# TritonDataCenter/dragnet

Measured on AMD Instinct MI355X. Metric: NDJSON records/sec (whole node), krill filter + 2-field breakdown (req.method,res.statusCode), higher is better.
Workload: dtype uint8; 1 GPU; model=dn scan: filter eq(req.method,GET) + breakdown req.method,res.statusCode, global_batch=4743501, seq_len=226, parallelism=dp1

## Files before the change

dragnet_amd/ops/hip/ext.hip:

```cpp

#include <torch/extension.h>
#include <cstdlib>
#include <cstring>
#include <c10/hip/HIPStream.h>

#include "scan_kernels.hip"

namespace dn {

namespace {

#define CHECK_GPU(t) TORCH_CHECK((t).is_cuda(), #t " must be on GPU")

constexpr size_t LDS_MAX = 160 * 1024;

hipStream_t current_stream() {
  return c10::hip::getCurrentHIPStream().stream();
}

template <class... KArgs, class... Args>
void launch(const char* what, void (*kernel)(KArgs...), dim3 grid,
            dim3 block, size_t lds, Args&&... args) {
  hipLaunchKernelGGL(kernel, grid, block, lds, current_stream(),
                     std::forward<Args>(args)...);
  hipError_t err = hipGetLastError();
  TORCH_CHECK(err == hipSuccess, what, " launch failed: ",
              hipGetErrorString(err));
}

uint32_t grid_for(uint64_t n) {
  return (uint32_t)std::min<uint64_t>((n + BLOCK - 1) / BLOCK, 2048);
}

int env_int(const char* name, int dflt) {
  const char* v = getenv(name);
  return v ? atoi(v) : dflt;
}

torch::Tensor tensor_at(const py::dict& d, const char* key) {
  return py::cast<torch::Tensor>(d[key]);
}

size_t lds_bytes(int64_t nf, int64_t nm, int64_t ns, bool columnar) {
  return LdsLayout((int)nf, (int)nm, columnar ? 0 : (int)ns, !columnar)
      .total;
}

using ScanKernel = void (*)(ScanArgs);

ScanKernel linear_kernel(int mw) {
  switch (mw) {
    case 2: return scan_kernel_mw<2>;
    case 3: return scan_kernel_mw<3>;
    case 4: return scan_kernel_mw<4>;
    case 5: return scan_kernel_mw<5>;
    case 6: return scan_kernel_mw<6>;
    default: return scan_kernel;
  }
}

ScanKernel xpose_kernel(int mw, int xg) {
  if (xg == 32) return scan_kernel_x<4, 5>;
  if (xg == 128) return scan_kernel_x<4, 7>;
  switch (mw) {
    case 2: return scan_kernel_x<2, 6>;
    case 3: return scan_kernel_x<3, 6>;
    case 5: return scan_kernel_x<5, 6>;
    default: return scan_kernel_x<4, 6>;
  }
}

}

void newline_index(torch::Tensor data, int64_t start, int64_t n,
                   torch::Tensor seg_scratch,
                   torch::Tensor pos_out, torch::Tensor total_out) {
  CHECK_GPU(data);
  int64_t span = n - (start & ~(int64_t)15);
  uint32_t nseg = (uint32_t)((span + NL_SEG - 1) / NL_SEG);
  TORCH_CHECK((int64_t)nseg <= seg_scratch.numel(),
              "seg_scratch too small");
  if (span <= 0) {
    total_out.zero_();
    return;
  }
  const uint8_t* d = (const uint8_t*)data.data_ptr();
  uint32_t* segs = (uint32_t*)seg_scratch.data_ptr();
  uint32_t blocks = (nseg + 3) / 4;
  launch("newline_count", newline_count_kernel, dim3(blocks), dim3(256), 0,
         d, (uint32_t)start, (uint32_t)n, segs, nseg);
  launch("newline_scan", newline_scan_kernel, dim3(1), dim3(1024), 0,
         segs, nseg, (uint32_t*)total_out.data_ptr());
  launch("newline_write", newline_write_kernel, dim3(blocks), dim3(256), 0,
         d, (uint32_t)start, (uint32_t)n, segs, nseg,
         (uint32_t*)pos_out.data_ptr(), (uint32_t)pos_out.numel());
}

torch::Tensor col_descs_host(std::vector<int64_t> kinds,
                             std::vector<torch::Tensor> nums,
                             std::vector<torch::Tensor> soffs,
                             std::vector<torch::Tensor> slens) {
  int nf = (int)kinds.size();
  auto out = torch::zeros({(long)(nf * sizeof(ColDesc))},
                          torch::dtype(torch::kUInt8));
  ColDesc* d = (ColDesc*)out.data_ptr();
  for (int f = 0; f < nf; f++) {
    d[f].kind = (int32_t)kinds[f];
    d[f].num = kinds[f] == 1 ? (const double*)nums[f].data_ptr()
                             : nullptr;
    d[f].soff = kinds[f] == 2 ? (const uint32_t*)soffs[f].data_ptr()
                              : nullptr;
    d[f].slen = kinds[f] == 2 ? (const uint32_t*)slens[f].data_ptr()
                              : nullptr;
  }
  return out;
}

void xpose_build(torch::Tensor data, torch::Tensor sstart,
                 torch::Tensor slen, torch::Tensor wbase,
                 int64_t n_slots, int64_t gran_log, torch::Tensor xb) {
  CHECK_GPU(data);
  CHECK_GPU(xb);
  uint32_t nw = (uint32_t)(n_slots >> 6);
  TORCH_CHECK(wbase.numel() >= (long)nw + 1, "wbase needs nw+1 rows");
  uint32_t blocks = (nw + 3) / 4;
  launch("xpose_build", xpose_build_kernel, dim3(blocks), dim3(256), 0,
         (const uint8_t*)data.data_ptr(),
         (const uint32_t*)sstart.data_ptr(),
         (const uint32_t*)slen.data_ptr(),
         (const unsigned long long*)wbase.data_ptr(),
         (uint32_t)n_slots, (int)gran_log, (uint8_t*)xb.data_ptr());
}

class ScanState {
 public:
  ScanState(py::dict plan, std::vector<torch::Tensor> states,
            std::vector<torch::Tensor> keys,
            std::vector<torch::Tensor> counts,
            std::vector<torch::Tensor> partials, py::dict sdict,
// ... 10 lines not shown
    StrDict& sd = args_.sdict;
    NumDict& nd = args_.ndict;
    P.field_sigs = (const uint64_t*)ptr(plan, "field_sigs");
    P.nf = (int)owned_.back().numel();
    P.comp_slot = (const int32_t*)ptr(plan, "comp_slot");
    P.nf_match = py::cast<int>(plan["nf_match"]);
    P.sig_bloom = (uint64_t)py::cast<int64_t>(plan["sig_bloom"]);
    P.prog_nodes = (const int32_t*)ptr(plan, "prog_nodes");
    P.prog_bounds = (const int32_t*)ptr(plan, "prog_bounds");
    P.const_meta = (const int32_t*)ptr(plan, "const_meta");
    P.const_dvals = (const double*)ptr(plan, "const_dvals");
    P.const_bytes = (const uint8_t*)ptr(plan, "const_bytes");
    P.synth_slots = (const int32_t*)ptr(plan, "synth_slots");
    P.ns = py::cast<int>(plan["n_synth"]);
    P.metric_rows = (const int32_t*)ptr(plan, "metric_rows");
    P.nm = (int)(owned_.back().numel() / 8);
    P.synth_req = (const int32_t*)ptr(plan, "synth_req");
    P.bd_rows = (const int32_t*)ptr(plan, "bd_rows");
    P.bd_steps = (const double*)ptr(plan, "bd_steps");
    P.value_slot = py::cast<int>(plan["value_slot"]);
    P.fields_slot = py::cast<int>(plan["fields_slot"]);
    P.fields_parent_sig =
        (uint64_t)py::cast<int64_t>(plan["fields_parent_sig"]);
    args_.data_format_skinner = py::cast<bool>(plan["skinner"]) ? 1 : 0;

    sd_state_ = tensor_at(sdict, "state");
    sd_data_ = tensor_at(sdict, "data");
    sd_used_ = tensor_at(sdict, "used");
    sd_next_ = tensor_at(sdict, "next");
    sd.state = (uint32_t*)sd_state_.data_ptr();
    sd.hash = (uint64_t*)ptr(sdict, "hash");
    sd.id = (uint32_t*)ptr(sdict, "id");
    sd.off = (uint32_t*)ptr(sdict, "off");
    sd.len = (uint32_t*)ptr(sdict, "len");
    sd.nslots = (uint32_t)sd_state_.numel();
    sd.data = (uint8_t*)sd_data_.data_ptr();
    sd.data_cap = (uint32_t)sd_data_.numel();
    sd.data_used = (uint32_t*)sd_used_.data_ptr();
    sd.next_id = (uint32_t*)sd_next_.data_ptr();

    nd_state_ = tensor_at(ndict, "state");
    nd_next_ = tensor_at(ndict, "next");
    nd.state = (uint32_t*)nd_state_.data_ptr();
    nd.bits = (uint64_t*)ptr(ndict, "bits");
    nd.id = (uint32_t*)ptr(ndict, "id");
    nd.nslots = (uint32_t)nd_state_.numel();
    nd.next_id = (uint32_t*)nd_next_.data_ptr();

    size_t nm = states_.size();
    TORCH_CHECK((int)nm == P.nm && keys_.size() == nm &&
                    counts_.size() == nm &&
                    (partials_.empty() || partials_.size() == nm),
                "one table (and partial) per metric");
    tables_.resize(nm);
    for (size_t m = 0; m < nm; m++) {
      AggTable& t = tables_[m];
      t.state = (uint32_t*)states_[m].data_ptr();
      t.keys = (uint32_t*)keys_[m].data_ptr();
      t.count = (double*)counts_[m].data_ptr();
      t.nslots = (uint32_t)states_[m].numel();
      t.partial = nullptr;
      t.prows = 0;
      t.pad_ = 0;
      if (!partials_.empty()) {
        TORCH_CHECK(partials_[m].size(1) == (long)t.nslots,
                    "partial width != nslots");
        t.partial = (double*)partials_[m].data_ptr();
        t.prows = (uint32_t)partials_[m].size(0);
      }
    }
    for (auto* group : {&states_, &keys_, &counts_, &partials_, &owned_})
      for (auto& t : *group) CHECK_GPU(t);
    for (auto* t : {&sd_state_, &sd_data_, &sd_used_, &sd_next_,
                    &nd_state_, &nd_next_})
      CHECK_GPU(*t);
    auto host = torch::empty({(long)(nm * sizeof(AggTable))},
                             torch::dtype(torch::kUInt8));
    memcpy(host.data_ptr(), tables_.data(), nm * sizeof(AggTable));
    table_descs_ = host.to(counters_.device());
    args_.tables = (AggTable*)table_descs_.data_ptr();
    args_.counters = (unsigned long long*)counters_.data_ptr();

    int mw = env_int("DRAGNET_MIN_WAVES", 4);
    linear_ = linear_kernel(mw);
    xpose_ = xpose_kernel(mw, env_int("DRAGNET_XGRAN", 64));

    lds_ = lds_bytes(P.nf, P.nm, P.ns, false);
    TORCH_CHECK(lds_ <= LDS_MAX, "plan needs too much LDS: ", lds_);
    int tile_req = env_int("DRAGNET_LDS_STAGE", 0);
    if (tile_req != 0) {
      size_t avail = (LDS_MAX - lds_ - 256) & ~(size_t)15;
      tile_cap_ = (tile_req < 0) ? avail
                                 : std::min((size_t)tile_req, avail);
      if (tile_cap_ > 100 * 1024) tile_cap_ = 100 * 1024;
      if (tile_cap_ < 24 * 1024) tile_cap_ = 0;
    }
    args_.tile_cap = (uint32_t)tile_cap_;
  }

  void scan(torch::Tensor data, torch::Tensor nl_pos,
            torch::Tensor nlines, int64_t first_start) {
    CHECK_GPU(data);
    CHECK_GPU(nl_pos);
    ScanArgs A = args_;
    A.data = (const uint8_t*)data.data_ptr();
    A.nl_pos = (const uint32_t*)nl_pos.data_ptr();
    A.nlines_ptr = (const uint32_t*)nlines.data_ptr();
    A.pos_cap = (uint32_t)nl_pos.numel();
    A.first_start = (uint32_t)first_start;
    launch("scan_kernel", linear_, dim3(grid_for(A.pos_cap)), dim3(BLOCK),
           lds_ + tile_cap_, A);
  }

  void scan_xpose(torch::Tensor xdata, torch::Tensor wave_base,
                  torch::Tensor rec_len, int64_t n_slots) {
    CHECK_GPU(xdata);
    TORCH_CHECK(n_slots > 0, "empty transposed staging");
    ScanArgs A = args_;
    A.xdata = (const uint8_t*)xdata.data_ptr();
    A.xwave_base = (const unsigned long long*)wave_base.data_ptr();
    A.xrec_len = (const uint32_t*)rec_len.data_ptr();
    A.xn_slots = (uint32_t)n_slots;
    launch("scan_kernel_x", xpose_, dim3(grid_for(A.xn_slots)),
           dim3(BLOCK), lds_ + tile_cap_, A);
  }

  void columnar_query(torch::Tensor col_descs, torch::Tensor blob,
                      torch::Tensor values, int64_t nrows,
                      std::vector<torch::Tensor> columns) {
    CHECK_GPU(col_descs);
    CHECK_GPU(blob);
    CHECK_GPU(values);
    for (auto& t : columns) CHECK_GPU(t);
    col_inputs_ = std::move(columns);
    col_inputs_.insert(col_inputs_.end(), {col_descs, blob, values});
    ColArgs A;
    A.nrows = (uint32_t)nrows;
    A.values = (const double*)values.data_ptr();
    A.blob = (const uint8_t*)blob.data_ptr();
    A.cols = (const ColDesc*)col_descs.data_ptr();
    A.P = args_.P;
    A.P.sig_bloom = 0;
    A.P.fields_parent_sig = 0;
    A.P.ns = 0;
    A.P.value_slot = -1;
    A.P.fields_slot = -1;
    A.tables = args_.tables;
    A.sdict = args_.sdict;
    A.ndict = args_.ndict;
    A.counters = args_.counters;
    size_t lds = lds_bytes(A.P.nf, A.P.nm, 0, true);
    TORCH_CHECK(lds <= LDS_MAX, "columnar plan needs too much LDS");
    uint32_t blocks = grid_for((uint64_t)nrows);
    if (blocks == 0) return;
    launch("columnar_query", columnar_query_kernel, dim3(blocks),
           dim3(BLOCK), lds, A);
  }

  void reset() {
    hipStream_t st = current_stream();
    auto z = [&](torch::Tensor& t) {
      hipError_t e = hipMemsetAsync(t.data_ptr(), 0,
                                    (size_t)t.numel() * t.element_size(),
                                    st);
      TORCH_CHECK(e == hipSuccess, "reset memset failed: ",
                  hipGetErrorString(e));
    };
    for (auto& t : states_) z(t);
    for (auto& t : counts_) z(t);
    for (auto& t : partials_) z(t);
    z(sd_state_); z(sd_used_); z(sd_next_);
    z(nd_state_); z(nd_next_); z(counters_);
  }

  std::vector<torch::Tensor> extract_all() {
    for (const AggTable& T : tables_) dense_reduce(T);
    const StrDict& sd = args_.sdict;
    const NumDict& nd = args_.ndict;
    auto i32 = torch::dtype(torch::kInt32).device(counters_.device());
    auto f64 = torch::dtype(torch::kFloat64).device(counters_.device());
// ... 96 lines not shown
```

dragnet_amd/ops/hip/scan_kernels.hip:

```cpp

#include "common.h"
#include <hip/hip_runtime.h>
#include "dec2dbl.h"

namespace dn {

#define DEV __device__ __forceinline__

constexpr int BLOCK = 256;
constexpr int SIG_DEPTH = 6;
constexpr int LDS_CACHE = 128;


DEV uint64_t fnv1a_byte(uint64_t h, uint8_t b) {
  return (h ^ (uint64_t)b) * 0x100000001B3ull;
}
constexpr uint64_t FNV_OFFSET = 0xCBF29CE484222325ull;

__device__ __constant__ double P10_TBL[23] = {
  1e0,1e1,1e2,1e3,1e4,1e5,1e6,1e7,1e8,1e9,1e10,1e11,1e12,1e13,1e14,
  1e15,1e16,1e17,1e18,1e19,1e20,1e21,1e22};
__device__ __constant__ int DIM_TBL[12] = {
  31,28,31,30,31,30,31,31,30,31,30,31};

DEV uint64_t mix64(uint64_t x) {
  x ^= x >> 33; x *= 0xFF51AFD7ED558CCDull;
  x ^= x >> 33; x *= 0xC4CEB9FE1A85EC53ull;
  x ^= x >> 33; return x;
}

#define DN_REGSEL6(T, NAME)                                            \
  struct NAME {                                                        \
    T a0, a1, a2, a3, a4, a5;                                          \
    DEV T get(int i) const {                                           \
      T r = a0;                                                        \
      r = (i == 1) ? a1 : r; r = (i == 2) ? a2 : r;                    \
      r = (i == 3) ? a3 : r; r = (i == 4) ? a4 : r;                    \
      r = (i == 5) ? a5 : r; return r;                                 \
    }                                                                  \
    DEV void set(int i, T x) {                                         \
      a0 = (i == 0) ? x : a0; a1 = (i == 1) ? x : a1;                  \
      a2 = (i == 2) ? x : a2; a3 = (i == 3) ? x : a3;                  \
      a4 = (i == 4) ? x : a4; a5 = (i == 5) ? x : a5;                  \
    }                                                                  \
  };
#define DN_REGSEL8(T, NAME)                                            \
  struct NAME {                                                        \
    T a0, a1, a2, a3, a4, a5, a6, a7;                                  \
    DEV T get(int i) const {                                           \
      T r = a0;                                                        \
      r = (i == 1) ? a1 : r; r = (i == 2) ? a2 : r;                    \
      r = (i == 3) ? a3 : r; r = (i == 4) ? a4 : r;                    \
      r = (i == 5) ? a5 : r; r = (i == 6) ? a6 : r;                    \
      r = (i == 7) ? a7 : r; return r;                                 \
    }                                                                  \
    DEV void set(int i, T x) {                                         \
      a0 = (i == 0) ? x : a0; a1 = (i == 1) ? x : a1;                  \
      a2 = (i == 2) ? x : a2; a3 = (i == 3) ? x : a3;                  \
      a4 = (i == 4) ? x : a4; a5 = (i == 5) ? x : a5;                  \
      a6 = (i == 6) ? x : a6; a7 = (i == 7) ? x : a7;                  \
    }                                                                  \
  };
DN_REGSEL6(uint64_t, Sig6)
DN_REGSEL8(uint64_t, U64x8)
DN_REGSEL8(double, F64x8)
DN_REGSEL8(uint32_t, U32x8)

template <typename T>
DEV T atomic_load_relaxed(const T* p) {
  return __hip_atomic_load(p, __ATOMIC_RELAXED, __HIP_MEMORY_SCOPE_AGENT);
}
template <typename T>
DEV void atomic_store_relaxed(T* p, T v) {
  __hip_atomic_store(p, v, __ATOMIC_RELAXED, __HIP_MEMORY_SCOPE_AGENT);
}
DEV void drain_stores() {
  asm volatile("s_waitcnt vmcnt(0)" ::: "memory");
}


struct Bytes {
  const uint8_t* mem;
  uint32_t bias;
  DEV uint8_t at(uint32_t abs) const { return mem[abs - bias]; }
  DEV const uint8_t* ptr(uint32_t abs) const { return mem + (abs - bias); }
  DEV uint64_t load8(uint32_t abs) const {
    uint64_t w;
    __builtin_memcpy(&w, mem + (abs - bias), 8);
    return w;
  }
};

template <int LG>
struct XBytesT {
  static constexpr uint32_t GRAN = 1u << LG;
  static constexpr uint32_t STRIDE = 64u << LG;
  const uint8_t* base;
  DEV uint8_t at(uint32_t p) const {
    return base[(size_t)(p >> LG) * STRIDE + (p & (GRAN - 1u))];
  }
  DEV uint64_t load8(uint32_t p) const {
    uint32_t o = p & (GRAN - 1u);
    const uint8_t* gp = base + (size_t)(p >> LG) * STRIDE;
    uint64_t w;
    if (o <= GRAN - 8) {
      __builtin_memcpy(&w, gp + o, 8);
      return w;
    }
    uint64_t lo, hi;
    __builtin_memcpy(&lo, gp + GRAN - 8, 8);
    __builtin_memcpy(&hi, gp + STRIDE, 8);
    uint32_t sh = (o - (GRAN - 8)) * 8;
    return (lo >> sh) | (hi << (64 - sh));
  }
};

template <class BS>
struct CursorT {
  BS B;
  uint32_t pos, end;
  uint64_t win, win2;
  uint32_t wbase;

  DEV void init(BS b, uint32_t p, uint32_t e) {
    B = b; pos = p; end = e;
    wbase = p;
    win = B.load8(p);
    win2 = B.load8(p + 8);
  }
  DEV uint8_t byte_at(uint32_t p) {
#ifdef DN_DIRECT_BYTES
    return B.at(p);
#else
    uint32_t d = p - wbase;
    if (d >= 16u) {
      wbase = p;
      win = B.load8(p);
      win2 = B.load8(p + 8);
      d = 0;
    }
    uint64_t w = d < 8u ? win : win2;
    return (uint8_t)(w >> (8u * (d & 7u)));
#endif
  }
  DEV bool eof() const { return pos >= end; }
  DEV uint8_t peek() { return byte_at(pos); }
  DEV uint8_t next() { return byte_at(pos++); }
  DEV uint64_t word_at(uint32_t p) {
#ifdef DN_DIRECT_BYTES
    return B.load8(p);
#else
    uint32_t d = p - wbase;
    if (d > 8u) {
      wbase = p;
      win = B.load8(p);
      win2 = B.load8(p + 8);
      d = 0;
    }
    if (d == 0) return win;
    if (d == 8u) return win2;
    return (win >> (8u * d)) | (win2 << (64u - 8u * d));
#endif
  }
  DEV void skip_ws() {
    while (pos < end) {
      uint8_t b = byte_at(pos);
      if (b == ' ' || b == '\t' || b == '\r' || b == '\n') pos++;
      else break;
    }
  }
};
using Cursor = CursorT<Bytes>;

DEV uint64_t hz8(uint64_t v) {
  return (v - 0x0101010101010101ull) & ~v & 0x8080808080808080ull;
}

DEV uint64_t str_special_mask(uint64_t w) {
  uint64_t q = hz8(w ^ 0x2222222222222222ull);
  uint64_t b = hz8(w ^ 0x5C5C5C5C5C5C5C5Cull);
  uint64_t c = hz8(w & 0xE0E0E0E0E0E0E0E0ull);
  return q | b | c;
}

template <class BS>
DEV bool scan_string_fast(CursorT<BS>& c, uint32_t& off_out,
                          uint32_t& len_out) {
  uint32_t off = c.pos, p = c.pos, end = c.end;
  while (true) {
    while (p + 8 <= end) {
      uint64_t w = c.B.load8(p);
      uint64_t m = str_special_mask(w);
      if (m == 0) { p += 8; continue; }
      p += ((uint32_t)__ffsll((unsigned long long)m) - 1) >> 3;
      break;
    }
    if (p >= end) return false;
    uint8_t b = c.B.at(p);
    if (b == '"') {
      off_out = off; len_out = p - off; c.pos = p + 1;
      return true;
    }
    if (b == '\\') {
      p++;
      if (p >= end) return false;
      uint8_t e = c.B.at(p); p++;
      if (e == 'u') {
        if (p + 4 > end) return false;
        for (int k = 0; k < 4; k++) {
          uint8_t x = c.B.at(p + k);
          bool hex = (x >= '0' && x <= '9') || (x >= 'a' && x <= 'f') ||
                     (x >= 'A' && x <= 'F');
          if (!hex) return false;
        }
        p += 4;
      } else if (!(e == '"' || e == '\\' || e == '/' || e == 'b' ||
                   e == 'f' || e == 'n' || e == 'r' || e == 't')) {
        return false;
      }
      continue;
    }
    if (b < 0x20) return false;
    p++;
  }
}

constexpr uint64_t SIG_LENK = 0xFF51AFD7ED558CCDull;

DEV inline uint64_t sig_mix(uint64_t x) {
  x ^= x >> 32;
  x *= 0xD6E8FEB86659FD93ull;
  return x ^ (x >> 32);
}
constexpr uint64_t SIG_LIT_MARK = 0xC2B2AE3D27D4EB4Full;

DEV inline uint64_t sig_word(uint64_t sig, uint64_t w) {
  return sig_mix(sig ^ w);
}
DEV inline uint64_t sig_fin(uint64_t sig, uint32_t len) {
  return sig_mix(sig ^ ((uint64_t)len * SIG_LENK));
}

template <class BS>
DEV uint64_t sig_comp_finish(BS B, uint64_t sig, uint32_t hashed,
                             uint32_t comp_s, uint32_t term) {
  uint32_t k = hashed;
  while (k < term) {
    uint64_t w = B.load8(k);
    uint32_t rem = term - k;
    if (rem < 8) w &= (~0ull) >> (8 * (8 - rem));
    sig = sig_mix(sig ^ w);
    k += 8;
  }
  return sig_fin(sig, term - comp_s);
}

template <class BS>
DEV int scan_key_sig(CursorT<BS>& c, uint64_t parent, uint64_t& sig_out,
                     bool dot_splits) {
  uint32_t p = c.pos, end = c.end;
  uint32_t comp_s = p;
  uint32_t hashed = p;
  uint64_t sig = parent;
  bool saw_dot = false;
  while (true) {
    while (p + 8 <= end) {
      uint64_t w = c.B.load8(p);
      uint64_t m = str_special_mask(w);
      if (dot_splits) m |= hz8(w ^ 0x2E2E2E2E2E2E2E2Eull);
      if (m == 0) {
        if (p == hashed) {
          sig = sig_word(sig, w);
          hashed = p + 8;
        }
        p += 8;
        continue;
      }
      p += ((uint32_t)__ffsll((unsigned long long)m) - 1) >> 3;
      break;
    }
    if (p >= end) return 0;
    uint8_t b = c.B.at(p);
    if (b == '"') {
      sig_out = sig_comp_finish(c.B, sig, hashed, comp_s, p);
      c.pos = p + 1;
      return saw_dot ? 2 : 1;
    }
    if (b == '.') {
      if (dot_splits) {
        sig = sig_comp_finish(c.B, sig, hashed, comp_s, p);
        comp_s = p + 1;
        hashed = p + 1;
        saw_dot = true;
      }
      p++;
      continue;
    }
    if (b == '\\') {
      c.pos = p;
      uint32_t o, l;
      if (!scan_string_fast(c, o, l)) return 0;
      sig_out = 0x1ull;
      return 1;
    }
    if (b < 0x20) return 0;
    p++;
  }
}


struct FV {
  uint8_t* type;
  uint32_t* soff;
  uint32_t* slen;
  int tid;
  DEV void set(int f, uint8_t t, uint32_t off, uint32_t len, double n) {
    type[f * BLOCK + tid] = t;
    if (t == T_NUM) {
      uint64_t b = (uint64_t)__double_as_longlong(n);
      soff[f * BLOCK + tid] = (uint32_t)b;
      slen[f * BLOCK + tid] = (uint32_t)(b >> 32);
    } else {
      soff[f * BLOCK + tid] = off;
      slen[f * BLOCK + tid] = len;
    }
  }
  DEV void set_len(int f, uint32_t len) { slen[f * BLOCK + tid] = len; }
  DEV uint8_t  get_type(int f) const { return type[f * BLOCK + tid]; }
  DEV uint32_t get_soff(int f) const { return soff[f * BLOCK + tid]; }
  DEV uint32_t get_slen(int f) const { return slen[f * BLOCK + tid]; }
  DEV double   get_num(int f) const {
    uint64_t b = (uint64_t)soff[f * BLOCK + tid]
               | ((uint64_t)slen[f * BLOCK + tid] << 32);
    return __longlong_as_double((long long)b);
  }
};


DEV double scale10(uint64_t mant, long ex) {
  return dn_dec2dbl(mant, ex, P10_TBL);
}

struct NumOut { double v; bool ok; };

template <class BS>
DEV int scan_digit_run(CursorT<BS>& c, uint64_t& mant, int& ndig,
                       int& extra) {
  int total = 0;
  while (!c.eof()) {
    uint64_t w = c.word_at(c.pos);
    uint64_t t = w ^ 0x3030303030303030ull;
    uint64_t nd = ((t + 0x7676767676767676ull) | t)
                  & 0x8080808080808080ull;
    uint32_t n = nd ? (((uint32_t)__ffsll((long long)nd) - 1) >> 3)
                    : 8u;
    uint32_t avail = c.end - c.pos;
    if (n > avail) n = avail;
    if (n == 0) break;
    if (n == 8 && mant != 0 && ndig + 8 <= 19) {
      uint64_t pairs = (t * ((10ull << 8) + 1)) >> 8;
      uint64_t quads = ((pairs & 0x00FF00FF00FF00FFull)
                        * ((100ull << 16) + 1)) >> 16;
      uint64_t v8 = ((quads & 0x0000FFFF0000FFFFull)
                     * ((10000ull << 32) + 1)) >> 32;
      mant = mant * 100000000ull + (uint32_t)v8;
      ndig += 8;
    } else {
      for (uint32_t k = 0; k < n; k++) {
        uint32_t d = (uint32_t)(w >> (8 * k)) & 0xFF;
        if (ndig < 19) {
          mant = mant * 10u + (d - '0');
          ndig += (mant != 0);
        } else extra++;
      }
    }
    c.pos += n;
    total += (int)n;
    if (n < 8) break;
// ... 1152 lines not shown
                                     uint32_t start, uint32_t n,
                                     const uint32_t* seg_offsets,
                                     uint32_t nseg, uint32_t* out_pos,
                                     uint32_t cap) {
  uint32_t seg = blockIdx.x * (blockDim.x >> 6) + (threadIdx.x >> 6);
  if (seg >= nseg) return;
  uint32_t lane = threadIdx.x & 63u;
  const uint4* p16 = reinterpret_cast<const uint4*>(data);
  uint32_t base0 = (start & ~15u) + seg * NL_SEG;
  uint32_t w_at = seg_offsets[seg];
#pragma unroll
  for (int half = 0; half < 2; half++) {
    uint32_t base = base0 + half * 1024u + lane * 16u;
    uint32_t m[4] = {0, 0, 0, 0};
    uint32_t cnt = 0;
    if (base < n) {
      uint4 v = p16[base >> 4];
      uint32_t w[4] = {v.x, v.y, v.z, v.w};
#pragma unroll
      for (int wi = 0; wi < 4; wi++) {
        m[wi] = nl_mask32(w[wi]) &
                range_mask32(base + wi * 4, start, n);
        cnt += __popc(m[wi]);
      }
    }
    uint32_t incl = cnt;
    for (int off = 1; off < 64; off <<= 1) {
      uint32_t t = __shfl_up(incl, off, 64);
      if ((int)lane >= off) incl += t;
    }
    uint32_t at = w_at + incl - cnt;
#pragma unroll
    for (int wi = 0; wi < 4; wi++) {
      uint32_t mm = m[wi];
      while (mm) {
        uint32_t b = ((uint32_t)__ffs(mm) - 1) >> 3;
        if (at < cap) out_pos[at] = base + wi * 4 + b;
        at++;
        mm &= mm - 1;
      }
    }
    w_at += __shfl(incl, 63, 64);
  }
}


struct ColDesc {
  int32_t kind;
  int32_t pad_;
  const double* num;
  const uint32_t* soff;
  const uint32_t* slen;
};

struct ColArgs {
  uint32_t nrows;
  const double* values;
  const uint8_t* blob;
  const ColDesc* cols;
  PlanView P;
  AggTable* tables;
  StrDict sdict;
  NumDict ndict;
  unsigned long long* counters;
};

__launch_bounds__(BLOCK, 5)
__global__ void columnar_query_kernel(ColArgs A) {
  extern __shared__ __attribute__((aligned(16))) char smemc[];
  const PlanView& P = A.P;
  const int nf = P.nf;
  const LdsLayout L(nf, P.nm, 0, false);
  LdsCacheEntry* cache = reinterpret_cast<LdsCacheEntry*>(smemc + L.cache);
  unsigned long long* lcnt =
      reinterpret_cast<unsigned long long*>(smemc + L.lcnt);
  const int NCNT = C_GLOBAL_N + P.nm * CM_N;
  block_agg_init(cache, lcnt, NCNT);

  FV fv;
  fv.type = reinterpret_cast<uint8_t*>(smemc + L.fv_type);
  fv.soff = reinterpret_cast<uint32_t*>(smemc + L.fv_soff);
  fv.slen = reinterpret_cast<uint32_t*>(smemc + L.fv_slen);
  fv.tid = threadIdx.x;
  Bytes BV;
  BV.mem = A.blob;
  BV.bias = 0;

  const uint32_t stride = gridDim.x * BLOCK;
  for (uint32_t r = blockIdx.x * BLOCK + threadIdx.x; r < A.nrows;
       r += stride) {
    atomicAdd(&lcnt[C_LINES], 1ull);
    atomicAdd(&lcnt[C_PARSED], 1ull);
    for (int f = 0; f < nf; f++) {
      const ColDesc& c = A.cols[f];
      if (c.kind == 1)
        fv.set(f, T_NUM, 0, 0, c.num[r]);
      else if (c.kind == 2)
        fv.set(f, T_STR, c.soff[r], c.slen[r], 0.0);
      else
        fv.set(f, T_MISSING, 0, 0, 0.0);
    }
    {
      int keep = eval_predicate(P, BV, fv, 0);
      if (keep != 1) {
        if (keep == -1) atomicAdd(&lcnt[C_DS_FAILEDEVAL], 1ull);
        else atomicAdd(&lcnt[C_DS_FILTERED], 1ull);
        continue;
      }
    }
    double weight = A.values[r];
    for (int m = 0; m < P.nm; m++) {
      const int32_t* M = &P.metric_rows[m * 8];
      unsigned long long* mc = &lcnt[C_GLOBAL_N + m * CM_N];
      atomicAdd(&mc[CM_AGG_IN], 1ull);

      uint32_t key[MAX_KEY];
      int nk = M[1];
      bool drop = false, overflow = false;
      for (int bi = 0; bi < nk; bi++) {
        const int32_t* B = &P.bd_rows[(M[2] + bi) * 4];
        int slot = B[1];
        uint32_t code;
        if (!encode_key_col(A.sdict, A.ndict, BV, fv.get_type(slot),
                            fv.get_num(slot), fv.get_soff(slot),
                            fv.get_slen(slot), B[2],
                            P.bd_steps[M[2] + bi], code, drop, overflow))
          break;
#pragma unroll
        for (int kk = 0; kk < MAX_KEY; kk++)
          if (kk == bi) key[kk] = code;
      }
      if (overflow) { atomicAdd(&lcnt[C_OVERFLOW], 1ull); continue; }
      if (drop) { atomicAdd(&mc[CM_NONNUMERIC], 1ull); continue; }
#pragma unroll
      for (int k = 0; k < MAX_KEY; k++)
        if (k >= nk) key[k] = 0;

      lds_cache_add<8>(cache, A.tables, A.counters, lcnt, m, key, nk,
                    agg_key_hash(m, key), weight);
    }
  }

  block_agg_flush(cache, lcnt, NCNT, P, A.tables, A.counters);
}

__global__ void xpose_build_kernel(const uint8_t* __restrict__ data,
                                   const uint32_t* __restrict__ sstart,
                                   const uint32_t* __restrict__ slen,
                                   const unsigned long long* __restrict__ wbase,
                                   uint32_t n_slots, int gran_log,
                                   uint8_t* __restrict__ xb) {
  uint32_t w = blockIdx.x * (blockDim.x >> 6) + (threadIdx.x >> 6);
  uint32_t nw = n_slots >> 6;
  if (w >= nw) return;
  uint32_t lane = threadIdx.x & 63u;
  uint32_t r = (w << 6) + lane;
  uint32_t gran = 1u << gran_log;
  unsigned long long base = wbase[w];
  uint32_t gw = (uint32_t)((wbase[w + 1] - base) >> (6 + gran_log));
  uint32_t len = slen[r];
  if (len == 0xFFFFFFFFu) len = 0;
  uint32_t start = sstart[r];
  uint8_t* dst0 = xb + base + ((size_t)lane << gran_log);
  for (uint32_t g = 0; g < gw; g++) {
    uint8_t* dst = dst0 + ((size_t)g << (6 + gran_log));
    uint32_t off = g << gran_log;
    for (uint32_t k = 0; k < gran; k += 16) {
      uint8_t tmp[16];
#pragma unroll
      for (int t = 0; t < 16; t++) {
        uint32_t o = off + k + t;
        tmp[t] = (o < len) ? data[start + o] : (uint8_t)'\n';
      }
      uint4 vv;
      __builtin_memcpy(&vv, tmp, 16);
      *reinterpret_cast<uint4*>(dst + k) = vv;
    }
  }
}

template <int XP>
DEV void scan_kernel_body(char* smem, ScanArgs A);

__launch_bounds__(BLOCK)
__global__ void scan_kernel(ScanArgs A) {
  extern __shared__ __attribute__((aligned(16))) char smem0[];
  scan_kernel_body<0>(smem0, A);
}

template <int MW>
__launch_bounds__(BLOCK, MW)
__global__ void scan_kernel_mw(ScanArgs A) {
  extern __shared__ __attribute__((aligned(16))) char smem1[];
  scan_kernel_body<0>(smem1, A);
}
template __global__ void scan_kernel_mw<2>(ScanArgs);
template __global__ void scan_kernel_mw<3>(ScanArgs);
template __global__ void scan_kernel_mw<4>(ScanArgs);
template __global__ void scan_kernel_mw<5>(ScanArgs);
template __global__ void scan_kernel_mw<6>(ScanArgs);

template <int MW, int XLG>
__launch_bounds__(BLOCK, MW)
__global__ void scan_kernel_x(ScanArgs A) {
  extern __shared__ __attribute__((aligned(16))) char smem2[];
  scan_kernel_body<XLG>(smem2, A);
}
template __global__ void scan_kernel_x<2, 6>(ScanArgs);
template __global__ void scan_kernel_x<3, 6>(ScanArgs);
template __global__ void scan_kernel_x<4, 6>(ScanArgs);
template __global__ void scan_kernel_x<5, 6>(ScanArgs);
template __global__ void scan_kernel_x<4, 5>(ScanArgs);
template __global__ void scan_kernel_x<4, 7>(ScanArgs);

#define synth_val_at(si) synth_lds[(si) * BLOCK + threadIdx.x]

template <class BS>
DEV void process_record(BS BV, uint32_t start, uint32_t end,
                        const ScanArgs& A, const PlanView& P, FV& fv,
                        unsigned long long* lcnt, LdsCacheEntry* cache,
                        uint64_t* sig_lds, double* synth_lds) {
  const int nf = P.nf;
  uint32_t synth_ok = 0;
  atomicAdd(&lcnt[C_LINES], 1ull);
  for (int f = 0; f < nf; f++)
    fv.type[f * BLOCK + fv.tid] = T_MISSING;

  uint8_t top_type;
  bool ok = (end > start) &&
            parse_record(BV, start, end, P, fv, top_type, sig_lds,
                         A.data_format_skinner);
  double weight = 1.0;
  if (ok && A.data_format_skinner) {
    bool has_fields = P.fields_slot >= 0 &&
                      fv.get_type(P.fields_slot) != T_MISSING;
    bool val_num = P.value_slot >= 0 &&
                   fv.get_type(P.value_slot) == T_NUM;
    if (top_type != T_OBJ || !has_fields || !val_num) ok = false;
    else weight = fv.get_num(P.value_slot);
  }
  if (!ok) {
    atomicAdd(&lcnt[C_INVALID_JSON], 1ull);
  } else {
    atomicAdd(&lcnt[C_PARSED], 1ull);

    int keep = eval_predicate(P, BV, fv, 0);
    if (keep == -1) atomicAdd(&lcnt[C_DS_FAILEDEVAL], 1ull);
    else if (keep == 0) atomicAdd(&lcnt[C_DS_FILTERED], 1ull);

    if (keep == 1) {
      synth_ok = 0;
      for (int si = 0; si < P.ns; si++) {
        int slot = P.synth_slots[si];
        uint8_t t = fv.get_type(slot);
        uint32_t ok;
        if (t == T_MISSING) ok = 2;
        else if (t == T_NUM) {
          ok = 1; synth_val_at(si) = fv.get_num(slot);
        } else if (t == T_STR) {
          DateOut d = parse_iso_ms(BV, fv.get_soff(slot),
                                   fv.get_slen(slot));
          if (d.ok) {
            long long secs = d.ms >= 0 ? d.ms / 1000
                                       : (d.ms - 999) / 1000;
            ok = 1; synth_val_at(si) = (double)secs;
          } else ok = 3;
        } else ok = 3;
        synth_ok |= ok << (2 * si);
      }

      for (int m = 0; m < P.nm; m++) {
        const int32_t* M = &P.metric_rows[m * 8];
        unsigned long long* mc = &lcnt[C_GLOBAL_N + m * CM_N];
        atomicAdd(&mc[CM_FILTER_IN], 1ull);

        int res = eval_predicate(P, BV, fv, M[0]);
        if (res == -1) { atomicAdd(&mc[CM_FAILEDEVAL], 1ull); continue; }
        if (res == 0) { atomicAdd(&mc[CM_FILTERED], 1ull); continue; }

        bool sok = true;
        for (int k = 0; k < M[3]; k++) {
          int si = P.synth_req[M[4] + k];
          uint32_t ok = (synth_ok >> (2 * si)) & 3u;
          if (ok != 1) {
            atomicAdd(&mc[ok == 2 ? CM_UNDEF : CM_BADDATE], 1ull);
            sok = false; break;
          }
        }
        if (!sok) continue;

        if (M[5]) {
          int si = P.synth_req[M[4] + M[3] - 1];
          double ts = synth_val_at(si);
          if (!(ts >= (double)M[6] && ts < (double)M[7])) {
            atomicAdd(&mc[CM_TIME_OUT], 1ull); continue;
          }
        }

        atomicAdd(&mc[CM_AGG_IN], 1ull);

        uint32_t key[MAX_KEY];
        int nk = M[1];
        bool drop = false, overflow = false;
        for (int bi = 0; bi < nk; bi++) {
          const int32_t* B = &P.bd_rows[(M[2] + bi) * 4];
          double step = P.bd_steps[M[2] + bi];
          uint8_t t; double num = 0.0; uint32_t so = 0, sl = 0;
          if (B[0] == 1) {
            int si = B[1];
            if (((synth_ok >> (2 * si)) & 3u) == 1) {
              t = T_NUM; num = synth_val_at(si);
            } else t = T_MISSING;
          } else {
            int slot = B[1];
            int cs2 = P.comp_slot[slot];
            if (cs2 >= 0 && fv.get_type(cs2) != T_MISSING)
              slot = cs2;
            t = fv.get_type(slot);
            num = fv.get_num(slot);
            so = fv.get_soff(slot); sl = fv.get_slen(slot);
          }
          uint32_t code;
          if (!encode_key_col(A.sdict, A.ndict, BV, t, num, so, sl, B[2],
                              step, code, drop, overflow))
            break;
#pragma unroll
          for (int kk = 0; kk < MAX_KEY; kk++)
            if (kk == bi) key[kk] = code;
        }
        if (overflow) { atomicAdd(&lcnt[C_OVERFLOW], 1ull); continue; }
        if (drop) { atomicAdd(&mc[CM_NONNUMERIC], 1ull); continue; }
#pragma unroll
        for (int k = 0; k < MAX_KEY; k++)
          if (k >= nk) key[k] = 0;

        uint64_t kh = agg_key_hash(m, key);

        if (!A.data_format_skinner) {
          uint64_t unproc = __ballot(true);
          bool leader = false;
          double wsum = 0.0;
          while (unproc) {
            int src = (int)(__ffsll((long long)unproc) - 1);
            uint64_t src_kh = __shfl(kh, src);
            bool same = (kh == src_kh);
            uint64_t grp = __ballot(same);
            if (same && __lane_id() == src) {
              leader = true;
              wsum = (double)__popcll(grp);
            }
            unproc &= ~grp;
          }
          if (!leader) continue;
          weight = wsum;
        }
        lds_cache_add<1>(cache, A.tables, A.counters, lcnt, m, key, nk, kh,
                      weight);
      }
    }
  }
}

template <int XP>
DEV void scan_kernel_body(char* smem, ScanArgs A) {
  const PlanView& P = A.P;
  const int nf = P.nf;

  const LdsLayout L(nf, P.nm, P.ns, true);
  LdsCacheEntry* cache = reinterpret_cast<LdsCacheEntry*>(smem + L.cache);
  unsigned long long* lcnt =
      reinterpret_cast<unsigned long long*>(smem + L.lcnt);
  const int NCNT = C_GLOBAL_N + P.nm * CM_N;
  double* synth_lds = reinterpret_cast<double*>(smem + L.synth);
  uint64_t* sig_lds = reinterpret_cast<uint64_t*>(smem + L.sig);
  uint8_t* tile = reinterpret_cast<uint8_t*>(smem + L.tile);
  block_agg_init(cache, lcnt, NCNT);

  FV fv;
  fv.type = reinterpret_cast<uint8_t*>(smem + L.fv_type);
  fv.soff = reinterpret_cast<uint32_t*>(smem + L.fv_soff);
  fv.slen = reinterpret_cast<uint32_t*>(smem + L.fv_slen);
  fv.tid = threadIdx.x;

  if constexpr (XP != 0) {
    const uint32_t stride_x = gridDim.x * BLOCK;
    for (uint32_t rbase = blockIdx.x * BLOCK; rbase < A.xn_slots;
         rbase += stride_x) {
      uint32_t r = rbase + threadIdx.x;
      if (r < A.xn_slots) {
        uint32_t len = A.xrec_len[r];
        if (len != 0xFFFFFFFFu) {
          XBytesT<XP> BV;
          BV.base = A.xdata + A.xwave_base[r >> 6]
                    + ((size_t)(r & 63u) << XP);
          process_record(BV, 0u, len, A, P, fv, lcnt, cache, sig_lds,
                         synth_lds);
        }
      }
    }
  } else {
  uint32_t nlines = *A.nlines_ptr;
  if (nlines > A.pos_cap) nlines = A.pos_cap;
  const uint32_t stride = gridDim.x * BLOCK;
  for (uint32_t rbase = blockIdx.x * BLOCK; rbase < nlines;
       rbase += stride) {
    uint32_t r = rbase + threadIdx.x;
    bool active = r < nlines;

    Bytes BV;
    BV.mem = A.data;
    BV.bias = 0;
    uint32_t t_start = rbase ? A.nl_pos[rbase - 1] + 1 : A.first_start;
    uint32_t r_last = rbase + BLOCK - 1;
    if (r_last >= nlines) r_last = nlines - 1;
    uint32_t t_end = A.nl_pos[r_last] + 1;
    uint32_t t_base = t_start & ~15u;
    uint32_t span = t_end - t_base;
    bool staged = A.tile_cap >= 16 && span <= A.tile_cap;
    if (staged) {
      const uint4* g16 = reinterpret_cast<const uint4*>(A.data + t_base);
      uint4* l16 = reinterpret_cast<uint4*>(tile);
      uint32_t n16 = (span + 15) >> 4;
      for (uint32_t i = threadIdx.x; i < n16; i += BLOCK)
        l16[i] = g16[i];
      __syncthreads();
      BV.mem = tile;
      BV.bias = t_base;
    }

    if (active) {
      uint32_t start = r ? A.nl_pos[r - 1] + 1 : A.first_start;
      uint32_t end = A.nl_pos[r];
      process_record(BV, start, end, A, P, fv, lcnt, cache, sig_lds,
                     synth_lds);
    }

    if (staged) __syncthreads();
  }
  }

  block_agg_flush(cache, lcnt, NCNT, P, A.tables, A.counters);
}


__global__ void extract_agg_kernel(AggTable T, uint32_t* out_keys,
                                   double* out_counts, uint32_t* out_n,
                                   uint32_t max_out) {
  uint32_t s = blockIdx.x * blockDim.x + threadIdx.x;
  if (s >= T.nslots) return;
  if (atomic_load_relaxed(&T.state[s]) != SLOT_READY) return;
  uint32_t i = atomicAdd(out_n, 1u);
  if (i >= max_out) return;
  for (int k = 0; k < MAX_KEY; k++)
    out_keys[i * MAX_KEY + k] = T.keys[s * MAX_KEY + k];
  out_counts[i] = T.count[s];
}

__global__ void extract_strdict_kernel(StrDict D, uint32_t* out_off,
                                       uint32_t* out_len, uint32_t max_ids) {
  uint32_t s = blockIdx.x * blockDim.x + threadIdx.x;
  if (s >= D.nslots) return;
  if (atomic_load_relaxed(&D.state[s]) != SLOT_READY) return;
  uint32_t id = D.id[s];
  if (id >= max_ids) return;
  out_off[id] = D.off[s];
  out_len[id] = D.len[s];
}

__global__ void extract_numdict_kernel(NumDict D, double* out_vals,
                                       uint32_t max_ids) {
  uint32_t s = blockIdx.x * blockDim.x + threadIdx.x;
  if (s >= D.nslots) return;
  if (atomic_load_relaxed(&D.state[s]) != SLOT_READY) return;
  uint32_t id = D.id[s];
  if (id >= max_ids) return;
  out_vals[id] = __longlong_as_double(
      (long long)atomic_load_relaxed(&D.bits[s]));
}

}
```

setup.py:

```python

import os

from setuptools import setup

os.environ.setdefault("PYTORCH_ROCM_ARCH", "gfx950")

import glob
import shutil

for stale in glob.glob("dragnet_amd/ops/hip/*_hip.hip"):
    os.unlink(stale)
shutil.rmtree("build/temp.linux-x86_64-3.10", ignore_errors=True)

import pybind11
from setuptools import Extension
from torch.utils.cpp_extension import BuildExtension, CUDAExtension

_SQLITE_SO = "/usr/lib/x86_64-linux-gnu/libsqlite3.so.0"

setup(
    name="dragnet_amd_ops",
    version="0.1.0",
    ext_modules=[
        CUDAExtension(
            name="dragnet_amd.ops._dragnet_hip",
            sources=["dragnet_amd/ops/hip/ext.hip"],
            extra_compile_args={
                "cxx": ["-O3", "-std=c++17"],
                "nvcc": [os.environ.get("DN_OPT", "-O3"), "-std=c++17"]
                        + (["-DDN_DIRECT_BYTES"]
                           if os.environ.get("DN_DIRECT_BYTES") else []),
            },
        ),
        Extension(
            name="dragnet_amd.index._points",
            sources=["dragnet_amd/index/points_fast.cpp"],
            include_dirs=[pybind11.get_include()],
            extra_compile_args=["-O3", "-std=c++17",
                                "-fvisibility=hidden"],
            language="c++",
        ),
        Extension(
            name="dragnet_amd.index._csink",
            sources=["dragnet_amd/index/csink.cpp"],
            include_dirs=[pybind11.get_include()],
            extra_compile_args=["-O3", "-std=c++17",
                                "-fvisibility=hidden"],
            extra_link_args=[_SQLITE_SO],
            language="c++",
        ),
    ],
    cmdclass={"build_ext": BuildExtension},
)
```

Before: 248.7 million records/s.

## Use address-space-typed byte loads, wave-aggregated counters, and a separate LDS tile kernel

```diff
diff --git a/dragnet_amd/ops/hip/ext.hip b/dragnet_amd/ops/hip/ext.hip
--- a/dragnet_amd/ops/hip/ext.hip
+++ b/dragnet_amd/ops/hip/ext.hip
@@ -48,13 +48,13 @@
 
 using ScanKernel = void (*)(ScanArgs);
 
-ScanKernel linear_kernel(int mw) {
+ScanKernel linear_kernel(int mw, bool tile) {
+  if (tile) return scan_kernel_tile;
   switch (mw) {
     case 2: return scan_kernel_mw<2>;
     case 3: return scan_kernel_mw<3>;
     case 4: return scan_kernel_mw<4>;
     case 5: return scan_kernel_mw<5>;
-    case 6: return scan_kernel_mw<6>;
     default: return scan_kernel;
   }
 }
@@ -231,8 +231,7 @@
     args_.counters = (unsigned long long*)counters_.data_ptr();
 
     int mw = env_int("DRAGNET_MIN_WAVES", 4);
-    linear_ = linear_kernel(mw);
-    xpose_ = xpose_kernel(mw, env_int("DRAGNET_XGRAN", 64));
+    xpose_ =xpose_kernel(mw, env_int("DRAGNET_XGRAN", 64));
 
     lds_ = lds_bytes(P.nf, P.nm, P.ns, false);
     TORCH_CHECK(lds_ <= LDS_MAX, "plan needs too much LDS: ", lds_);
@@ -245,6 +244,7 @@
       if (tile_cap_ < 24 * 1024) tile_cap_ = 0;
     }
     args_.tile_cap = (uint32_t)tile_cap_;
+    linear_ = linear_kernel(mw, tile_cap_ != 0);
   }
 
   void scan(torch::Tensor data, torch::Tensor nl_pos,
diff --git a/dragnet_amd/ops/hip/scan_kernels.hip b/dragnet_amd/ops/hip/scan_kernels.hip
--- a/dragnet_amd/ops/hip/scan_kernels.hip
+++ b/dragnet_amd/ops/hip/scan_kernels.hip
@@ -79,15 +79,37 @@
 }
 
 
-struct Bytes {
-  const uint8_t* mem;
+#define DN_AS_GLOBAL __attribute__((address_space(1)))
+#define DN_AS_LDS __attribute__((address_space(3)))
+typedef const DN_AS_GLOBAL uint8_t* gbytes_t;
+typedef const DN_AS_LDS uint8_t* lbytes_t;
+typedef uint64_t dn_u64_u __attribute__((aligned(1)));
+typedef uint64_t dn_u64x2_u
+    __attribute__((ext_vector_type(2), aligned(1)));
+
+struct GBytes {
+  gbytes_t mem;
+  DEV uint8_t at(uint32_t abs) const { return mem[abs]; }
+  DEV uint64_t load8(uint32_t abs) const {
+    return *reinterpret_cast<const DN_AS_GLOBAL dn_u64_u*>(mem + abs);
+  }
+  DEV void load16(uint32_t abs, uint64_t& lo, uint64_t& hi) const {
+    dn_u64x2_u v =
+        *reinterpret_cast<const DN_AS_GLOBAL dn_u64x2_u*>(mem + abs);
+    lo = v.x; hi = v.y;
+  }
+};
+
+struct LBytes {
+  lbytes_t mem;
   uint32_t bias;
   DEV uint8_t at(uint32_t abs) const { return mem[abs - bias]; }
-  DEV const uint8_t* ptr(uint32_t abs) const { return mem + (abs - bias); }
   DEV uint64_t load8(uint32_t abs) const {
-    uint64_t w;
-    __builtin_memcpy(&w, mem + (abs - bias), 8);
-    return w;
+    return *reinterpret_cast<const DN_AS_LDS dn_u64_u*>(
+        mem + (abs - bias));
+  }
+  DEV void load16(uint32_t abs, uint64_t& lo, uint64_t& hi) const {
+    lo = load8(abs); hi = load8(abs + 8);
   }
 };
 
@@ -95,23 +117,24 @@
 struct XBytesT {
   static constexpr uint32_t GRAN = 1u << LG;
   static constexpr uint32_t STRIDE = 64u << LG;
-  const uint8_t* base;
+  gbytes_t base;
   DEV uint8_t at(uint32_t p) const {
     return base[(size_t)(p >> LG) * STRIDE + (p & (GRAN - 1u))];
   }
   DEV uint64_t load8(uint32_t p) const {
     uint32_t o = p & (GRAN - 1u);
-    const uint8_t* gp = base + (size_t)(p >> LG) * STRIDE;
-    uint64_t w;
-    if (o <= GRAN - 8) {
-      __builtin_memcpy(&w, gp + o, 8);
-      return w;
-    }
-    uint64_t lo, hi;
-    __builtin_memcpy(&lo, gp + GRAN - 8, 8);
-    __builtin_memcpy(&hi, gp + STRIDE, 8);
+    gbytes_t gp = base + (size_t)(p >> LG) * STRIDE;
+    if (o <= GRAN - 8)
+      return *reinterpret_cast<const DN_AS_GLOBAL dn_u64_u*>(gp + o);
+    uint64_t lo = *reinterpret_cast<const DN_AS_GLOBAL dn_u64_u*>(
+        gp + GRAN - 8);
+    uint64_t hi = *reinterpret_cast<const DN_AS_GLOBAL dn_u64_u*>(
+        gp + STRIDE);
     uint32_t sh = (o - (GRAN - 8)) * 8;
     return (lo >> sh) | (hi << (64 - sh));
+  }
+  DEV void load16(uint32_t p, uint64_t& lo, uint64_t& hi) const {
+    lo = load8(p); hi = load8(p + 8);
   }
 };
 
@@ -125,42 +148,31 @@
   DEV void init(BS b, uint32_t p, uint32_t e) {
     B = b; pos = p; end = e;
     wbase = p;
-    win = B.load8(p);
-    win2 = B.load8(p + 8);
+    B.load16(p, win, win2);
   }
   DEV uint8_t byte_at(uint32_t p) {
-#ifdef DN_DIRECT_BYTES
-    return B.at(p);
-#else
     uint32_t d = p - wbase;
     if (d >= 16u) {
       wbase = p;
-      win = B.load8(p);
-      win2 = B.load8(p + 8);
+      B.load16(p, win, win2);
       d = 0;
     }
     uint64_t w = d < 8u ? win : win2;
     return (uint8_t)(w >> (8u * (d & 7u)));
-#endif
   }
   DEV bool eof() const { return pos >= end; }
   DEV uint8_t peek() { return byte_at(pos); }
   DEV uint8_t next() { return byte_at(pos++); }
   DEV uint64_t word_at(uint32_t p) {
-#ifdef DN_DIRECT_BYTES
-    return B.load8(p);
-#else
     uint32_t d = p - wbase;
     if (d > 8u) {
       wbase = p;
-      win = B.load8(p);
-      win2 = B.load8(p + 8);
+      B.load16(p, win, win2);
       d = 0;
     }
     if (d == 0) return win;
     if (d == 8u) return win2;
     return (win >> (8u * d)) | (win2 << (64u - 8u * d));
-#endif
   }
   DEV void skip_ws() {
     while (pos < end) {
@@ -170,7 +182,6 @@
     }
   }
 };
-using Cursor = CursorT<Bytes>;
 
 DEV uint64_t hz8(uint64_t v) {
   return (v - 0x0101010101010101ull) & ~v & 0x8080808080808080ull;
@@ -188,15 +199,18 @@
                           uint32_t& len_out) {
   uint32_t off = c.pos, p = c.pos, end = c.end;
   while (true) {
+    uint32_t inhand = 256;
     while (p + 8 <= end) {
       uint64_t w = c.B.load8(p);
       uint64_t m = str_special_mask(w);
       if (m == 0) { p += 8; continue; }
-      p += ((uint32_t)__ffsll((unsigned long long)m) - 1) >> 3;
+      uint32_t idx = ((uint32_t)__ffsll((unsigned long long)m) - 1) >> 3;
+      p += idx;
+      inhand = (uint32_t)(w >> (8u * idx)) & 0xFFu;
       break;
     }
     if (p >= end) return false;
-    uint8_t b = c.B.at(p);
+    uint8_t b = inhand < 256 ? (uint8_t)inhand : c.B.at(p);
     if (b == '"') {
       off_out = off; len_out = p - off; c.pos = p + 1;
       return true;
@@ -264,6 +278,9 @@
   uint64_t sig = parent;
   bool saw_dot = false;
   while (true) {
+    uint32_t inhand = 256;
+    uint64_t tailw = 0;
+    bool tail_ok = false;
     while (p + 8 <= end) {
       uint64_t w = c.B.load8(p);
       uint64_t m = str_special_mask(w);
@@ -276,24 +293,33 @@
         p += 8;
         continue;
       }
-      p += ((uint32_t)__ffsll((unsigned long long)m) - 1) >> 3;
+      uint32_t idx = ((uint32_t)__ffsll((unsigned long long)m) - 1) >> 3;
+      inhand = (uint32_t)(w >> (8u * idx)) & 0xFFu;
+      if (p == hashed) {
+        tail_ok = true;
+        tailw = idx ? (w & (~0ull >> (64u - 8u * idx))) : 0ull;
+      }
+      p += idx;
       break;
     }
     if (p >= end) return 0;
-    uint8_t b = c.B.at(p);
-    if (b == '"') {
-      sig_out = sig_comp_finish(c.B, sig, hashed, comp_s, p);
-      c.pos = p + 1;
-      return saw_dot ? 2 : 1;
-    }
-    if (b == '.') {
-      if (dot_splits) {
+    uint8_t b = inhand < 256 ? (uint8_t)inhand : c.B.at(p);
+    if (b == '"' || (b == '.' && dot_splits)) {
+      if (tail_ok) {
+        if (p != hashed) sig = sig_mix(sig ^ tailw);
+        sig = sig_fin(sig, p - comp_s);
+      } else {
         sig = sig_comp_finish(c.B, sig, hashed, comp_s, p);
-        comp_s = p + 1;
-        hashed = p + 1;
-        saw_dot = true;
+      }
+      if (b == '"') {
+        sig_out = sig;
+        c.pos = p + 1;
+        return saw_dot ? 2 : 1;
       }
       p++;
+      comp_s = p;
+      hashed = p;
+      saw_dot = true;
       continue;
     }
     if (b == '\\') {
@@ -1612,9 +1638,8 @@
   fv.soff = reinterpret_cast<uint32_t*>(smemc + L.fv_soff);
   fv.slen = reinterpret_cast<uint32_t*>(smemc + L.fv_slen);
   fv.tid = threadIdx.x;
-  Bytes BV;
-  BV.mem = A.blob;
-  BV.bias = 0;
+  GBytes BV;
+  BV.mem = (gbytes_t)A.blob;
 
   const uint32_t stride = gridDim.x * BLOCK;
   for (uint32_t r = blockIdx.x * BLOCK + threadIdx.x; r < A.nrows;
@@ -1709,32 +1734,37 @@
   }
 }
 
-template <int XP>
+template <int XP, bool TILE>
 DEV void scan_kernel_body(char* smem, ScanArgs A);
 
 __launch_bounds__(BLOCK)
 __global__ void scan_kernel(ScanArgs A) {
   extern __shared__ __attribute__((aligned(16))) char smem0[];
-  scan_kernel_body<0>(smem0, A);
+  scan_kernel_body<0, false>(smem0, A);
 }
 
 template <int MW>
 __launch_bounds__(BLOCK, MW)
 __global__ void scan_kernel_mw(ScanArgs A) {
   extern __shared__ __attribute__((aligned(16))) char smem1[];
-  scan_kernel_body<0>(smem1, A);
+  scan_kernel_body<0, false>(smem1, A);
 }
 template __global__ void scan_kernel_mw<2>(ScanArgs);
 template __global__ void scan_kernel_mw<3>(ScanArgs);
 template __global__ void scan_kernel_mw<4>(ScanArgs);
 template __global__ void scan_kernel_mw<5>(ScanArgs);
-template __global__ void scan_kernel_mw<6>(ScanArgs);
+
+__launch_bounds__(BLOCK, 3)
+__global__ void scan_kernel_tile(ScanArgs A) {
+  extern __shared__ __attribute__((aligned(16))) char smem3[];
+  scan_kernel_body<0, true>(smem3, A);
+}
 
 template <int MW, int XLG>
 __launch_bounds__(BLOCK, MW)
 __global__ void scan_kernel_x(ScanArgs A) {
   extern __shared__ __attribute__((aligned(16))) char smem2[];
-  scan_kernel_body<XLG>(smem2, A);
+  scan_kernel_body<XLG, false>(smem2, A);
 }
 template __global__ void scan_kernel_x<2, 6>(ScanArgs);
 template __global__ void scan_kernel_x<3, 6>(ScanArgs);
@@ -1744,6 +1774,16 @@
 template __global__ void scan_kernel_x<4, 7>(ScanArgs);
 
 #define synth_val_at(si) synth_lds[(si) * BLOCK + threadIdx.x]
+
+DEV void wave_count(unsigned long long* p) {
+  uint32_t a = (uint32_t)(uintptr_t)p;
+  uint32_t a0 = (uint32_t)__builtin_amdgcn_readfirstlane((int)a);
+  uint64_t grp = __ballot(a == a0);
+  if (a != a0)
+    atomicAdd(p, 1ull);
+  else if ((int)__lane_id() == __ffsll((long long)grp) - 1)
+    atomicAdd(p, (unsigned long long)__popcll(grp));
+}
 
 template <class BS>
 DEV void process_record(BS BV, uint32_t start, uint32_t end,
@@ -1752,7 +1792,7 @@
                         uint64_t* sig_lds, double* synth_lds) {
   const int nf = P.nf;
   uint32_t synth_ok = 0;
-  atomicAdd(&lcnt[C_LINES], 1ull);
+  wave_count(&lcnt[C_LINES]);
   for (int f = 0; f < nf; f++)
     fv.type[f * BLOCK + fv.tid] = T_MISSING;
 
@@ -1770,13 +1810,13 @@
     else weight = fv.get_num(P.value_slot);
   }
   if (!ok) {
-    atomicAdd(&lcnt[C_INVALID_JSON], 1ull);
+    wave_count(&lcnt[C_INVALID_JSON]);
   } else {
-    atomicAdd(&lcnt[C_PARSED], 1ull);
+    wave_count(&lcnt[C_PARSED]);
 
     int keep = eval_predicate(P, BV, fv, 0);
-    if (keep == -1) atomicAdd(&lcnt[C_DS_FAILEDEVAL], 1ull);
-    else if (keep == 0) atomicAdd(&lcnt[C_DS_FILTERED], 1ull);
+    if (keep == -1) wave_count(&lcnt[C_DS_FAILEDEVAL]);
+    else if (keep == 0) wave_count(&lcnt[C_DS_FILTERED]);
 
     if (keep == 1) {
       synth_ok = 0;
@@ -1802,11 +1842,11 @@
       for (int m = 0; m < P.nm; m++) {
         const int32_t* M = &P.metric_rows[m * 8];
         unsigned long long* mc = &lcnt[C_GLOBAL_N + m * CM_N];
-        atomicAdd(&mc[CM_FILTER_IN], 1ull);
+        wave_count(&mc[CM_FILTER_IN]);
 
         int res = eval_predicate(P, BV, fv, M[0]);
-        if (res == -1) { atomicAdd(&mc[CM_FAILEDEVAL], 1ull); continue; }
-        if (res == 0) { atomicAdd(&mc[CM_FILTERED], 1ull); continue; }
+        if (res == -1) { wave_count(&mc[CM_FAILEDEVAL]); continue; }
+        if (res == 0) { wave_count(&mc[CM_FILTERED]); continue; }
 
         bool sok = true;
         for (int k = 0; k < M[3]; k++) {
@@ -1823,11 +1863,11 @@
           int si = P.synth_req[M[4] + M[3] - 1];
           double ts = synth_val_at(si);
           if (!(ts >= (double)M[6] && ts < (double)M[7])) {
-            atomicAdd(&mc[CM_TIME_OUT], 1ull); continue;
+            wave_count(&mc[CM_TIME_OUT]); continue;
           }
         }
 
-        atomicAdd(&mc[CM_AGG_IN], 1ull);
+        wave_count(&mc[CM_AGG_IN]);
 
         uint32_t key[MAX_KEY];
         int nk = M[1];
@@ -1859,7 +1899,7 @@
             if (kk == bi) key[kk] = code;
         }
         if (overflow) { atomicAdd(&lcnt[C_OVERFLOW], 1ull); continue; }
-        if (drop) { atomicAdd(&mc[CM_NONNUMERIC], 1ull); continue; }
+        if (drop) { wave_count(&mc[CM_NONNUMERIC]); continue; }
 #pragma unroll
         for (int k = 0; k < MAX_KEY; k++)
           if (k >= nk) key[k] = 0;
@@ -1891,7 +1931,7 @@
   }
 }
 
-template <int XP>
+template <int XP, bool TILE>
 DEV void scan_kernel_body(char* smem, ScanArgs A) {
   const PlanView& P = A.P;
   const int nf = P.nf;
@@ -1904,6 +1944,7 @@
   double* synth_lds = reinterpret_cast<double*>(smem + L.synth);
   uint64_t* sig_lds = reinterpret_cast<uint64_t*>(smem + L.sig);
   uint8_t* tile = reinterpret_cast<uint8_t*>(smem + L.tile);
+  (void)tile;
   block_agg_init(cache, lcnt, NCNT);
 
   FV fv;
@@ -1921,7 +1962,7 @@
         uint32_t len = A.xrec_len[r];
         if (len != 0xFFFFFFFFu) {
           XBytesT<XP> BV;
-          BV.base = A.xdata + A.xwave_base[r >> 6]
+          BV.base = (gbytes_t)A.xdata + A.xwave_base[r >> 6]
                     + ((size_t)(r & 63u) << XP);
           process_record(BV, 0u, len, A, P, fv, lcnt, cache, sig_lds,
                          synth_lds);
@@ -1937,35 +1978,45 @@
     uint32_t r = rbase + threadIdx.x;
     bool active = r < nlines;
 
-    Bytes BV;
-    BV.mem = A.data;
-    BV.bias = 0;
-    uint32_t t_start = rbase ? A.nl_pos[rbase - 1] + 1 : A.first_start;
-    uint32_t r_last = rbase + BLOCK - 1;
-    if (r_last >= nlines) r_last = nlines - 1;
-    uint32_t t_end = A.nl_pos[r_last] + 1;
-    uint32_t t_base = t_start & ~15u;
-    uint32_t span = t_end - t_base;
-    bool staged = A.tile_cap >= 16 && span <= A.tile_cap;
-    if (staged) {
-      const uint4* g16 = reinterpret_cast<const uint4*>(A.data + t_base);
-      uint4* l16 = reinterpret_cast<uint4*>(tile);
-      uint32_t n16 = (span + 15) >> 4;
-      for (uint32_t i = threadIdx.x; i < n16; i += BLOCK)
-        l16[i] = g16[i];
-      __syncthreads();
-      BV.mem = tile;
-      BV.bias = t_base;
-    }
-
+    uint32_t start = 0, end = 0;
     if (active) {
-      uint32_t start = r ? A.nl_pos[r - 1] + 1 : A.first_start;
-      uint32_t end = A.nl_pos[r];
-      process_record(BV, start, end, A, P, fv, lcnt, cache, sig_lds,
-                     synth_lds);
-    }
-
-    if (staged) __syncthreads();
+      start = r ? A.nl_pos[r - 1] + 1 : A.first_start;
+      end = A.nl_pos[r];
+    }
+    GBytes GV;
+    GV.mem = (gbytes_t)A.data;
+
+    if constexpr (TILE) {
+      uint32_t t_start = rbase ? A.nl_pos[rbase - 1] + 1 : A.first_start;
+      uint32_t r_last = rbase + BLOCK - 1;
+      if (r_last >= nlines) r_last = nlines - 1;
+      uint32_t t_end = A.nl_pos[r_last] + 1;
+      uint32_t t_base = t_start & ~15u;
+      uint32_t span = t_end - t_base;
+      bool staged = A.tile_cap >= 16 && span <= A.tile_cap;
+      if (staged) {
+        const uint4* g16 = reinterpret_cast<const uint4*>(A.data + t_base);
+        uint4* l16 = reinterpret_cast<uint4*>(tile);
+        uint32_t n16 = (span + 15) >> 4;
+        for (uint32_t i = threadIdx.x; i < n16; i += BLOCK)
+          l16[i] = g16[i];
+        __syncthreads();
+        LBytes LV;
+        LV.mem = (lbytes_t)tile;
+        LV.bias = t_base;
+        if (active)
+          process_record(LV, start, end, A, P, fv, lcnt, cache, sig_lds,
+                         synth_lds);
+        __syncthreads();
+      } else if (active) {
+        process_record(GV, start, end, A, P, fv, lcnt, cache, sig_lds,
+                       synth_lds);
+      }
+    } else {
+      if (active)
+        process_record(GV, start, end, A, P, fv, lcnt, cache, sig_lds,
+                       synth_lds);
+    }
   }
   }
 
diff --git a/setup.py b/setup.py
--- a/setup.py
+++ b/setup.py
@@ -27,9 +27,7 @@
             sources=["dragnet_amd/ops/hip/ext.hip"],
             extra_compile_args={
                 "cxx": ["-O3", "-std=c++17"],
-                "nvcc": [os.environ.get("DN_OPT", "-O3"), "-std=c++17"]
-                        + (["-DDN_DIRECT_BYTES"]
-                           if os.environ.get("DN_DIRECT_BYTES") else []),
+                "nvcc": [os.environ.get("DN_OPT", "-O3"), "-std=c++17"],
             },
         ),
         Extension(
```

Result: no change. 248.7 million records/s, median of 2 (+0.0%).
